# katie-jones/compressor-mpc

Measured on AMD Instinct MI355X. Metric: QP solves/sec (whole node), cooperative-parallel MPC, horizon p=50, higher is better.
Workload: dtype f64

## Files before the change

### compressor-mpc_amd/csrc/build_pair_kernel.h

```cpp
#pragma once
#include <hip/hip_runtime.h>
#include <stdint.h>

#include <algorithm>

#include "dispatch.h"
#include "rows_blocks.inc"

#ifndef CMPC_PAIR_ZDEPTH
#define CMPC_PAIR_ZDEPTH 1
#endif
static_assert(CMPC_PAIR_ZDEPTH == 1 || CMPC_PAIR_ZDEPTH == 2, "CMPC_PAIR_ZDEPTH");

__device__ __forceinline__ void pair_wait_dma() {
  asm volatile("" ::: "memory");
  __builtin_amdgcn_s_waitcnt(0x0F70);
  asm volatile("" ::: "memory");
}

template <int NS, int NY, int NUT, int NU, int M, int ND>
__global__ __launch_bounds__(64 * CMPC_BUILD_WAVES) __attribute__((amdgpu_waves_per_eu(2, 2)))
void cmpc_build_pair_kernel(BuildParams P) {
  extern __shared__ __attribute__((aligned(16))) double smem[];
  constexpr int WPG = CMPC_BUILD_WAVES;
  constexpr int NV = NU * M;
  constexpr int NC = M * NUT;
  constexpr int NG = NC + 2;
  constexpr int U = cmpc_rows_unroll(NY);
  constexpr int NCMP = CMPC_PAIR_CMP;
  static_assert(U == 5, "the unrolled block has 5 steps");
  static_assert(M == 2 && ND == 2 && NUT == 2 * NU, "two sub-controllers, two delayed inputs");
  static_assert(NG <= 16 && NS + NUT <= 16 && NS + NY + ND <= 16, "lane budget");
  const int lane = threadIdx.x & 63;
  const int wave = __builtin_amdgcn_readfirstlane(threadIdx.x >> 6);
  const int R = lane >> 4, j = lane & 15;
  const int pp = P.p, nobs = P.nobs, rl = P.rec_len, ndist = P.ndist;
  const int LQ = P.rows.LQ, WL = P.pair.WL, yls = P.rows.yls;
  const int nscn = P.nqp >> 1;
  const int ngroups = (nscn + 3) / 4;
  const int nwaves = gridDim.x * WPG;

  double* zeros = smem;
  double* ylT = smem + P.rows.yl_off;
  double* lw_all = smem + P.rows.lw_off;
  double* uw_all = smem + P.rows.uw_off;
  double* wreg = smem + P.rows.lds_block + wave * P.pair.per_wave;
  double* lines = wreg;
  double* chs = wreg + P.rows.ch_off;
  double* z1s = wreg + P.pair.z1_off;
  double* wtab = wreg + P.pair.w_off;

  const int nthr = 64 * WPG;
  for (int e = threadIdx.x; e < 2 * NY * yls; e += nthr) {
    const int ss = e / (NY * yls), rem = e - ss * NY * yls;
    const int o = rem / yls, r = rem - o * yls;
    ylT[e] = (r < pp) ? -P.cfg[(size_t)ss * P.co.len + P.co.yhat + r * NY + o] : 0.0;
  }
  for (int e = threadIdx.x; e < 2 * NY * NY; e += nthr)
    lw_all[e] = P.cfg[(size_t)(e / (NY * NY)) * P.co.len + P.co.lwt + e % (NY * NY)];
  for (int e = threadIdx.x; e < 2 * NU * NU; e += nthr)
    uw_all[e] = P.cfg[(size_t)(e / (NU * NU)) * P.co.len + P.co.uwt + e % (NU * NU)];
  if (threadIdx.x < 16) zeros[threadIdx.x] = 0.0;
  for (int e = lane; e < P.pair.per_wave; e += 64) wreg[e] = 0.0;
  if (blockIdx.x == 0 && threadIdx.x == 0) *P.pair_cnt_next = 0u;
  __syncthreads();

  const bool st = j < NS;
  const bool mk = j >= NS && j < NS + NUT;
  const int cm = mk ? j - NS : 0;
  const bool ol = j >= NS && j < NS + NY;
  const int oo = ol ? j - NS : 0;
  const bool cl = j >= 16 - ND;
  const int kc = cl ? j - (16 - ND) : 0;
  const bool gl = j < NG;
  const bool zl0 = j == NC, zl1 = j == NC + 1, zlane = zl0 || zl1;
  const int gk = (gl && !zlane) ? j / NUT : 0;
  const int gc = (gl && !zlane) ? j - gk * NUT : 0;
  const double smask = (gl && !zlane && gk == M - 1) ? 1.0 : 0.0;
  int dg = 0, dm = 0, log_ = 0, lom = 0, dinp[ND], dlen[ND], boff[ND];
#pragma unroll
  for (int c = 0; c < NUT; ++c) {
    if (c == gc) { dg = P.delay[c]; log_ = P.rows.lo[c]; }
    if (c == cm) { dm = P.delay[c]; lom = P.rows.lo[c]; }
  }
#pragma unroll
  for (int k = 0; k < ND; ++k) {
    dinp[k] = P.dinput[k];
    dlen[k] = P.dlen[k];
    boff[k] = P.boff[k];
  }
  int ysw = -1;
#pragma unroll
  for (int k = 0; k < ND; ++k)
    if (cl && k == kc && dlen[k] < pp) ysw = dlen[k];
  const int nseg = P.rows.nseg;
  constexpr int NSEG = 2 * ND;
  int segb[NSEG];
#pragma unroll
  for (int i = 0; i < NSEG; ++i) segb[i] = P.rows.seg[i];
  double* const qlines = lines + R * LQ;
  const bool rdel = gl && !zlane && dg > 0;
  const int rsw = (rdel && dg < pp) ? dg : -1;
  double* const zrow = qlines + P.rows.zr_off;
  double* const r_start = !gl ? zrow
                          : zl0 ? qlines + P.rows.z_off
                          : zl1 ? z1s + R * U * NY
                          : (dg == 0) ? qlines + log_ + (1 - gk) * NY
                                      : zrow;
  double* const r_line = qlines + log_ + (M - 1 - gk) * NY;
  const bool wdel = mk && dm > 0;
  double* const dump = qlines + P.rows.dump_off;
  double* const w_start = !mk ? dump
                          : (dm == 0) ? qlines + lom + NY
                          : (pp - dm > 0) ? qlines + lom + (M - 1) * NY
                                          : dump;
  const int winc0 = (wdel && pp - dm > 0) ? NY : 0;
  const int wsw = (wdel && pp - dm > 0) ? pp - dm : -1;
  const bool tl = mk && dm == 0;
  double* const tq = qlines + lom;
  double* const zq0 = ol ? qlines + P.rows.z_off + oo : dump;
  double* const zq1 = ol ? z1s + R * U * NY + oo : dump;

  const int t0 = P.pair.tail0, wch = rl >> 1, tch = (rl - t0) >> 1, sps = 2 * rl - t0;
  const int hd = P.off_x;
  int pli[NCMP];
#pragma unroll
  for (int i = 0; i < NCMP; ++i) {
    const int idx = 64 * i + lane;
    pli[i] = idx;
    if (idx >= P.off_B && idx < P.off_C) {
      const int t = idx - P.off_B, l = t / NUT, c = t - l * NUT;
      pli[i] = P.off_B + l * NUT + (c + NU) % NUT;
    }
  }

  const int share = (ngroups + nwaves - 1) / nwaves;
  const int g_first = blockIdx.x * WPG + wave;
  int done_groups = 0;
  uint32_t shared_scn = 0;
  __builtin_amdgcn_s_setprio(3);
  for (int g = g_first; g < ngroups; g += nwaves) {
    {
      const int level = 3 - (4 * done_groups) / share;
      if (level <= 0) __builtin_amdgcn_s_setprio(0);
      else if (level == 1) __builtin_amdgcn_s_setprio(1);
      else if (level == 2) __builtin_amdgcn_s_setprio(2);
      ++done_groups;
    }
    const int scn = 4 * g + R;
    const bool qv = scn < nscn;
    const int scc = qv ? scn : nscn - 1;
    const int nsc = min(4, nscn - 4 * g);
    const double* gbase = P.lin + (size_t)8 * g * rl;
    auto stage = [&](int h) {
#pragma unroll
      for (int sc = 0; sc < 4; ++sc) {
        if (sc >= nsc) break;
        const double* rec = gbase + (2 * sc + h) * rl + 2 * lane;
        const double* tal = gbase + (2 * sc + 1 - h) * rl + t0 + 2 * lane;
        double* dst = wreg + sc * sps;
        auto* gp = (__attribute__((address_space(1))) void*)rec;
        auto* lp = (__attribute__((address_space(3))) void*)dst;
        if (wch >= 64) __builtin_amdgcn_global_load_lds(gp, lp, 16, 0, 0);
        else if (lane < wch) __builtin_amdgcn_global_load_lds(gp, lp, 16, 0, 0);
        if (wch >= 128) __builtin_amdgcn_global_load_lds(gp, lp, 16, 1024, 0);
        else if (lane < wch - 64) __builtin_amdgcn_global_load_lds(gp, lp, 16, 1024, 0);
        if (wch >= 192) __builtin_amdgcn_global_load_lds(gp, lp, 16, 2048, 0);
        else if (lane < wch - 128) __builtin_amdgcn_global_load_lds(gp, lp, 16, 2048, 0);
        if (lane < tch)
          __builtin_amdgcn_global_load_lds((__attribute__((address_space(1))) void*)tal,
                                           (__attribute__((address_space(3))) void*)(dst + rl), 16, 0, 0);
      }
    };
    const double* lwt = lw_all;

    asm volatile("s_waitcnt lgkmcnt(0)" ::: "memory");
    stage(0);
    uint64_t hv[4][NCMP];
#pragma unroll
    for (int sc = 0; sc < 4; ++sc) {
      const int scl = min(sc, nsc - 1);
#pragma unroll
      for (int i = 0; i < NCMP; ++i)
        hv[sc][i] = reinterpret_cast<const uint64_t*>(gbase + (2 * scl + 1) * rl + 64 * i)[(uint32_t)lane];
    }
    double uo[2][ND], dyr[2][NY];
#pragma unroll
    for (int s = 0; s < 2; ++s) {
#pragma unroll
      for (int k = 0; k < ND; ++k) uo[s][k] = P.u_old[(size_t)(2 * scc + s) * NUT + dinp[k]];
#pragma unroll
      for (int o2 = 0; o2 < NY; ++o2) dyr[s][o2] = 0.0;
    }
    if (P.dy_ref) {
      uint32_t qo = (uint32_t)(2 * scc) * NY;
      asm volatile("" : "+v"(qo));
#pragma unroll
      for (int s = 0; s < 2; ++s)
#pragma unroll
        for (int o2 = 0; o2 < NY; ++o2) dyr[s][o2] = P.dy_ref[qo + s * NY + o2];
    }
    pair_wait_dma();
    uint64_t diff = 0ull;
#pragma unroll
    for (int sc = 0; sc < 4; ++sc) {
      const uint64_t* s0 = reinterpret_cast<const uint64_t*>(wreg + min(sc, nsc - 1) * sps);
#pragma unroll
      for (int i = 0; i < NCMP; ++i) {
        const uint64_t x = hv[sc][i] ^ s0[pli[i]];
        diff |= (64 * i + lane < hd) ? x : 0ull;
      }
    }
    const bool mism = __ballot(diff != 0ull) != 0ull;
    if (!mism) shared_scn += (uint32_t)nsc;

    for (int h = 0;; ++h) {
      int jg = j, Rg = R;
      asm volatile("" : "+v"(jg), "+v"(Rg));
      double* chq = chs + Rg * NY * 16;
      const double* srec = wreg + Rg * sps;
      const int rot = h * NU;
      const double *xa[2], *yv[2];
#pragma unroll
      for (int s = 0; s < 2; ++s) {
        const double* tb = (s == h) ? srec : srec + rl - t0;
        xa[s] = tb + P.off_x;
        yv[s] = tb + P.off_y;
      }
#pragma unroll
      for (int s = 0; s < 2; ++s)
#pragma unroll
        for (int k = 0; k < ND; ++k) {
          double* wk = wtab + ((Rg * 2 + s) * ND + k) * WL;
#pragma unroll
          for (int i = 0; i < 4; ++i) {
            const int t = jg + 16 * i;
            if (t < WL)
              wk[t] = (t < dlen[k]) ? ((t == 0) ? xa[s][ndist + k] : xa[s][boff[k] + t - 1]) - uo[s][k] : 0.0;
          }
        }
      double cs[NY];
#pragma unroll
      for (int o2 = 0; o2 < NY; ++o2) cs[o2] = (j < nobs) ? srec[P.off_C + o2 * nobs + jg] : 0.0;
      constexpr int KX = 16 - NS;
      double kx[2][KX], ky[2][NY];
#pragma unroll
      for (int s = 0; s < 2; ++s) {
#pragma unroll
        for (int d = 0; d < KX; ++d) kx[s][d] = (d < ndist) ? xa[s][d] : 0.0;
#pragma unroll
        for (int o2 = 0; o2 < NY; ++o2) ky[s][o2] = yv[s][o2];
#pragma unroll
        for (int o2 = 0; o2 < NY; ++o2) ky[s][o2] = ky[s][o2] - dyr[s][o2];
      }
      double mP[NS];
      if (st) {
        const double* src = srec + P.off_A + jg;
#pragma unroll
        for (int l = 0; l < NS; ++l) mP[l] = src[l * NS];
      } else if (mk) {
        const double* src = srec + P.off_B + (cm + rot) % NUT;
#pragma unroll
        for (int l = 0; l < NS; ++l) mP[l] = src[l * NUT];
      } else {
#pragma unroll
        for (int l = 0; l < NS; ++l) mP[l] = 0.0;
      }
      double mS[NS + ND], fj = 0.0;
      if (st) {
        const double* arow = srec + P.off_A + jg * NS;
        const double* brow = srec + P.off_B + jg * NUT;
#pragma unroll
        for (int l = 0; l < NS; ++l) mS[l] = arow[l];
#pragma unroll
        for (int k = 0; k < ND; ++k) mS[NS + k] = brow[(dinp[k] + rot) % NUT];
        fj = srec[P.off_f + jg];
      } else {
#pragma unroll
        for (int l = 0; l < NS + ND; ++l) mS[l] = 0.0;
      }
      __builtin_amdgcn_sched_barrier(0);

      double pP[NY];
#pragma unroll
      for (int o = 0; o < NY; ++o) {
        double t = 0.0;
#pragma unroll
        for (int o2 = 0; o2 < NY; ++o2)
          if (o2 >= o) t = __builtin_fma(lwt[o * NY + o2], cs[o2], t);
        if (j < nobs) chq[o * 16 + jg] = t;
        pP[o] = st ? t : 0.0;
      }
      double base0 = 0.0, base1 = 0.0, pS0 = 0.0, pS1 = 0.0, yh0 = 0.0, yh1 = 0.0;
      const double *yp0 = zeros, *yp1 = zeros;
      int yinc = 0;
      if (st) {
        base0 = base1 = fj;
        pS0 = pS1 = fj;
#pragma unroll
        for (int k = 0; k < ND; ++k) {
          pS0 = __builtin_fma(mS[NS + k], wtab[((Rg * 2 + 0) * ND + k) * WL], pS0);
          pS1 = __builtin_fma(mS[NS + ND - 1 - k], wtab[((Rg * 2 + 1) * ND + k) * WL], pS1);
        }
      } else if (ol) {
#pragma unroll
        for (int l = 0; l < NS; ++l) mS[l] = chq[oo * 16 + l];
        double t[2] = {0.0, 0.0};
#pragma unroll
        for (int s = 0; s < 2; ++s) {
#pragma unroll
          for (int d = 0; d < KX; ++d)
            if (d < ndist) t[s] = __builtin_fma(chq[oo * 16 + NS + d], kx[s][d], t[s]);
#pragma unroll
          for (int o2 = 0; o2 < NY; ++o2)
            if (o2 >= oo) t[s] = __builtin_fma(lwt[oo * NY + o2], ky[s][o2], t[s]);
        }
        base0 = t[0];
        base1 = t[1];
        const double* yl = ylT + oo * yls;
        yh0 = yl[0];
        yh1 = yl[NY * yls];
        yp0 = yl + 1;
        yp1 = yl + NY * yls + 1;
        yinc = 1;
      } else if (cl) {
        const double* wk0 = wtab + ((Rg * 2 + 0) * ND + kc) * WL;
        const double* wk1 = wtab + ((Rg * 2 + 1) * ND + (ND - 1 - kc)) * WL;
        pS0 = wk0[1];
        yh0 = wk0[2];
        yp0 = wk0 + 3;
        pS1 = wk1[1];
        yh1 = wk1[2];
        yp1 = wk1 + 3;
        yinc = 1;
      }
#pragma unroll
      for (int c = 0; c < NUT; ++c)
        if (P.delay[c] > 0 && j < (M - 1) * NY) qlines[P.rows.lo[c] + j] = 0.0;
      for (int e = j; e < U * NY; e += 16) qlines[P.rows.zr_off + e] = 0.0;
      if (tl) {
#pragma unroll
        for (int o = 0; o < NY; ++o) tq[o] = 0.0;
      }
      double cv[NY], rd[NY], acc[NC];
#pragma unroll
      for (int o = 0; o < NY; ++o) cv[o] = rd[o] = 0.0;
#pragma unroll
      for (int a = 0; a < NC; ++a) acc[a] = 0.0;
      double* wq = w_start;
      double* rq = r_start;
      int winc = winc0, rinc = 0;

#define CMPC_PAIR_STEP(u)                                                                  \
  {                                                                                        \
    double aS0 = aN0, aS1 = aN1;                                                           \
    yh0 = yp0[u];                                                                          \
    yh1 = yp1[u];                                                                          \
    double aP[NY];                                                                         \
    _Pragma("unroll") for (int o = 0; o < NY; ++o) aP[o] = z1[o];                          \
    rows_pair_head<NS, NY, ND, NUT, M>(pP, pS0, pS1, mP, mS, aP, aS0, aS1, cv, acc);       \
    __builtin_amdgcn_sched_barrier(0);                                                     \
    _Pragma("unroll") for (int o = 0; o < NY; ++o) cv[o] = __builtin_fma(smask, cv[o], rd[o]); \
    __builtin_amdgcn_sched_barrier(0);                                                     \
    rows_pair_part0<NS, NY, ND, NUT, M>(pP, pS0, pS1, mP, mS, aP, aS0, aS1, cv, acc);      \
    rows_pair_part1<NS, NY, ND, NUT, M>(pP, pS0, pS1, mP, mS, aP, aS0, aS1, cv, acc);      \
    __builtin_amdgcn_sched_barrier(0);                                                     \
    _Pragma("unroll") for (int o = 0; o < NY; ++o) pP[o] = aP[o];                          \
    pS0 = aS0;                                                                             \
    pS1 = aS1;                                                                             \
    if constexpr (CMPC_PAIR_ZDEPTH == 2) {                                                 \
      _Pragma("unroll") for (int o = 0; o < NY; ++o) z1[o] = z2[o];                        \
      _Pragma("unroll") for (int o = 0; o < NY; ++o) z2[o] = zeros[o];                     \
    } else {                                                                               \
      _Pragma("unroll") for (int o = 0; o < NY; ++o) z1[o] = zeros[o];                     \
    }                                                                                      \
    _Pragma("unroll") for (int o = 0; o < NY; ++o) wq[(u) * NY + o] = aP[o];               \
    zq0[(u) * NY] = aS0;                                                                   \
    zq1[(u) * NY] = aS1;                                                                   \
    _Pragma("unroll") for (int o = 0; o < NY; ++o) rd[o] = rq[(u) * NY + o];               \
    aN0 = base0 + yh0;                                                                     \
    aN1 = base1 + yh1;                                                                     \
    __builtin_amdgcn_sched_barrier(0);                                                     \
  }
#define CMPC_PAIR_TAIL()                                        \
  if (tl) {                                                     \
    _Pragma("unroll") for (int o = 0; o < NY; ++o) tq[o] = pP[o]; \
  }

      int r = 0;
      double aN0 = base0 + yh0, aN1 = base1 + yh1;
      double z1[NY], z2[NY];
#pragma unroll
      for (int o = 0; o < NY; ++o) z1[o] = z2[o] = zeros[o];
      for (int sg = 0; sg <= nseg; ++sg) {
        int r_end = pp;
#pragma unroll
        for (int i = 0; i < NSEG; ++i)
          if (i == sg && sg < nseg) r_end = segb[i];
        for (; r + U <= r_end; r += U) {
          CMPC_PAIR_STEP(0)
          CMPC_PAIR_STEP(1)
          CMPC_PAIR_STEP(2)
          CMPC_PAIR_STEP(3)
          CMPC_PAIR_STEP(4)
          CMPC_PAIR_TAIL()
          wq += U * winc;
          rq += U * rinc;
          yp0 += U * yinc;
          yp1 += U * yinc;
        }
        while (r + 2 <= r_end) {
          CMPC_PAIR_STEP(0)
          CMPC_PAIR_STEP(1)
          CMPC_PAIR_TAIL()
          wq += 2 * winc;
          rq += 2 * rinc;
          yp0 += 2 * yinc;
          yp1 += 2 * yinc;
          r += 2;
        }
        for (; r < r_end; ++r) {
          CMPC_PAIR_STEP(0)
          CMPC_PAIR_TAIL()
          wq += winc;
          rq += rinc;
          yp0 += yinc;
          yp1 += yinc;
        }
        if (r == rsw) { rq = r_line; rinc = NY; }
        if (r == wsw) { wq = dump; winc = 0; }
        if (r == ysw) { yp0 = yp1 = zeros; yinc = 0; }
      }
#undef CMPC_PAIR_STEP
#undef CMPC_PAIR_TAIL
#pragma unroll
      for (int o = 0; o < NY; ++o) cv[o] = __builtin_fma(smask, cv[o], rd[o]);
      rows_pair_gacc<NY, NUT, M>(cv, acc);

      if (qv && gl) {
        constexpr int nuo = NUT - NU, nVo = M * nuo;
        const int k2 = j / NUT, c2 = j - k2 * NUT;
#pragma unroll
        for (int s = 0; s < 2; ++s) {
          if (mism && s != h) continue;
          double* out = P.qp + (size_t)(2 * scn + s) * P.qp_len;
          const double* uwt = uw_all + s * NU * NU;
          double own[NV];
#pragma unroll
          for (int a = 0; a < NV; ++a) own[a] = acc[(a / NU) * NUT + (a % NU + s * NU) % NUT];
          if (zlane) {
            if (j == NC + s) {
#pragma unroll
              for (int a = 0; a < NV; ++a) out[NV * NV + a] = own[a];
            }
          } else {
            const int cs_ = (c2 + NUT - s * NU) % NUT;
            if (cs_ < NU) {
#pragma unroll
              for (int a = 0; a < NV; ++a) {
                const double rw = (a / NU == k2) ? uwt[(a % NU) * NU + cs_] : 0.0;
                out[a * NV + k2 * NU + cs_] = own[a] + rw;
              }
            } else {
#pragma unroll
              for (int a = 0; a < NV; ++a) out[NV * NV + NV + a * nVo + k2 * nuo + (cs_ - NU)] = own[a];
            }
          }
        }
      }
      __builtin_amdgcn_wave_barrier();
      if (!mism || h == 1) break;
      asm volatile("s_waitcnt lgkmcnt(0)" ::: "memory");
      stage(1);
      pair_wait_dma();
    }
  }
  if (lane == 0 && shared_scn) atomicAdd(P.pair_cnt, shared_scn);
}

template <int NS, int NY, int NU, int M>
static int pair_launch(const BuildParams& P, hipStream_t s) {
  auto kern = cmpc_build_pair_kernel<NS, NY, CMPC_DIMS_NUT, NU, M, CMPC_DIMS_ND>;
  constexpr int WPG = CMPC_BUILD_WAVES;
  const size_t lds = sizeof(double) * ((size_t)P.rows.lds_block + (size_t)P.pair.per_wave * WPG);
  if (lds > 64 * 1024) cmpc_allow_lds(reinterpret_cast<const void*>(kern), lds);
  const int per_cu = 2;
  const int nscn = P.nqp / 2;
  const int need = std::max(1, ((nscn + 3) / 4 + WPG - 1) / WPG);
  const int grid = std::max(1, std::min(need, P.cus * per_cu));
  cmpc_launch(kern, dim3(grid), dim3(64 * WPG), lds, s, P);
  return 0;
}
```

Before: 4.642 billion.

## Branch-free pair setup with hoisted loads and high priority during setup

Rewrites the per-half setup of the pair build kernel so it has no branches. Loads are issued with pointer selects, redirecting to a zero buffer or dump slot instead of using conditional paths, and all operand loads are hoisted ahead of a scheduling barrier so their latency overlaps. By default the wave now holds top priority through setup and only drops to its fair-share priority when the main row loop starts. The change also adds opt-in timing instrumentation and a next-group prefetch touch, both disabled by default. Risks are extra register pressure from hoisting and extra dummy stores.

Measured after the change: 4.792 billion (median of 6 runs). 3.2% higher.

```diff
diff --git a/compressor-mpc_amd/csrc/build_pair_kernel.h b/compressor-mpc_amd/csrc/build_pair_kernel.h
--- a/compressor-mpc_amd/csrc/build_pair_kernel.h
+++ b/compressor-mpc_amd/csrc/build_pair_kernel.h
@@ -11,6 +11,28 @@
 #define CMPC_PAIR_ZDEPTH 1
 #endif
 static_assert(CMPC_PAIR_ZDEPTH == 1 || CMPC_PAIR_ZDEPTH == 2, "CMPC_PAIR_ZDEPTH");
+
+#ifndef CMPC_PAIR_TIMING
+#define CMPC_PAIR_TIMING 0
+#endif
+#ifndef CMPC_PAIR_SETUP_PRIO
+#define CMPC_PAIR_SETUP_PRIO 1
+#endif
+#ifndef CMPC_PAIR_TOUCH
+#define CMPC_PAIR_TOUCH 0
+#endif
+#if CMPC_PAIR_TIMING
+#define CMPC_PT(i)                                         \
+  {                                                        \
+    __builtin_amdgcn_sched_barrier(0);                     \
+    const uint64_t now_ = __builtin_amdgcn_s_memtime();    \
+    tsum[i] += now_ - tlast;                               \
+    tlast = now_;                                          \
+    __builtin_amdgcn_sched_barrier(0);                     \
+  }
+#else
+#define CMPC_PT(i)
+#endif
 
 __device__ __forceinline__ void pair_wait_dma() {
   asm volatile("" ::: "memory");
@@ -138,36 +160,45 @@
   const int g_first = blockIdx.x * WPG + wave;
   int done_groups = 0;
   uint32_t shared_scn = 0;
+#if CMPC_PAIR_TIMING
+  uint64_t tsum[7] = {0, 0, 0, 0, 0, 0, 0}, tlast = __builtin_amdgcn_s_memtime();
+  const uint64_t t0c = tlast, t0r = __builtin_amdgcn_s_memrealtime();
+  int ngrp = 0;
+#endif
   __builtin_amdgcn_s_setprio(3);
+  float touch[3] = {0.f, 0.f, 0.f};
   for (int g = g_first; g < ngroups; g += nwaves) {
-    {
-      const int level = 3 - (4 * done_groups) / share;
+    CMPC_PT(6)
+    const int level = 3 - (4 * done_groups) / share;
+    ++done_groups;
+    auto fair_prio = [&]() {
       if (level <= 0) __builtin_amdgcn_s_setprio(0);
       else if (level == 1) __builtin_amdgcn_s_setprio(1);
       else if (level == 2) __builtin_amdgcn_s_setprio(2);
-      ++done_groups;
-    }
+    };
+    if (CMPC_PAIR_SETUP_PRIO) __builtin_amdgcn_s_setprio(3);
+    else fair_prio();
     const int scn = 4 * g + R;
     const bool qv = scn < nscn;
     const int scc = qv ? scn : nscn - 1;
     const int nsc = min(4, nscn - 4 * g);
     const double* gbase = P.lin + (size_t)8 * g * rl;
-    auto stage = [&](int h) {
+    auto stage = [&](int h, int ln) {
 #pragma unroll
       for (int sc = 0; sc < 4; ++sc) {
         if (sc >= nsc) break;
-        const double* rec = gbase + (2 * sc + h) * rl + 2 * lane;
-        const double* tal = gbase + (2 * sc + 1 - h) * rl + t0 + 2 * lane;
+        const double* rec = gbase + (2 * sc + h) * rl + 2 * ln;
+        const double* tal = gbase + (2 * sc + 1 - h) * rl + t0 + 2 * ln;
         double* dst = wreg + sc * sps;
         auto* gp = (__attribute__((address_space(1))) void*)rec;
         auto* lp = (__attribute__((address_space(3))) void*)dst;
         if (wch >= 64) __builtin_amdgcn_global_load_lds(gp, lp, 16, 0, 0);
-        else if (lane < wch) __builtin_amdgcn_global_load_lds(gp, lp, 16, 0, 0);
+        else if (ln < wch) __builtin_amdgcn_global_load_lds(gp, lp, 16, 0, 0);
         if (wch >= 128) __builtin_amdgcn_global_load_lds(gp, lp, 16, 1024, 0);
-        else if (lane < wch - 64) __builtin_amdgcn_global_load_lds(gp, lp, 16, 1024, 0);
+        else if (ln < wch - 64) __builtin_amdgcn_global_load_lds(gp, lp, 16, 1024, 0);
         if (wch >= 192) __builtin_amdgcn_global_load_lds(gp, lp, 16, 2048, 0);
-        else if (lane < wch - 128) __builtin_amdgcn_global_load_lds(gp, lp, 16, 2048, 0);
-        if (lane < tch)
+        else if (ln < wch - 128) __builtin_amdgcn_global_load_lds(gp, lp, 16, 2048, 0);
+        if (ln < tch)
           __builtin_amdgcn_global_load_lds((__attribute__((address_space(1))) void*)tal,
                                            (__attribute__((address_space(3))) void*)(dst + rl), 16, 0, 0);
       }
@@ -175,7 +206,7 @@
     const double* lwt = lw_all;
 
     asm volatile("s_waitcnt lgkmcnt(0)" ::: "memory");
-    stage(0);
+    stage(0, lane);
     uint64_t hv[4][NCMP];
 #pragma unroll
     for (int sc = 0; sc < 4; ++sc) {
@@ -200,7 +231,10 @@
 #pragma unroll
         for (int o2 = 0; o2 < NY; ++o2) dyr[s][o2] = P.dy_ref[qo + s * NY + o2];
     }
+    CMPC_PT(0)
     pair_wait_dma();
+    CMPC_PT(1)
+    if (CMPC_PAIR_TOUCH) asm volatile("" ::"v"(touch[0]), "v"(touch[1]), "v"(touch[2]));
     uint64_t diff = 0ull;
 #pragma unroll
     for (int sc = 0; sc < 4; ++sc) {
@@ -213,6 +247,7 @@
     }
     const bool mism = __ballot(diff != 0ull) != 0ull;
     if (!mism) shared_scn += (uint32_t)nsc;
+    CMPC_PT(2)
 
     for (int h = 0;; ++h) {
       int jg = j, Rg = R;
@@ -227,6 +262,67 @@
         xa[s] = tb + P.off_x;
         yv[s] = tb + P.off_y;
       }
+      static_assert(U * NY <= 16, "one zero-restore store per lane");
+      static_assert((NUT & (NUT - 1)) == 0, "column rotation by a mask");
+      const int oog = ol ? jg - NS : 0, kcg = cl ? jg - (16 - ND) : 0, cmg = mk ? jg - NS : 0;
+      double wv[2][ND][4];
+      bool wlive[ND][4];
+#pragma unroll
+      for (int k = 0; k < ND; ++k)
+#pragma unroll
+        for (int i = 0; i < 4; ++i) {
+          const int t = jg + 16 * i;
+          wlive[k][i] = t < WL && t < dlen[k];
+          const int src = (wlive[k][i] && t > 0) ? boff[k] + t - 1 : ndist + k;
+#pragma unroll
+          for (int s = 0; s < 2; ++s) wv[s][k][i] = xa[s][src];
+        }
+      const bool jo = j < nobs;
+      double cs[NY];
+      {
+        const double* src = jo ? srec + P.off_C + jg : zeros;
+        const int str = jo ? nobs : 0;
+#pragma unroll
+        for (int o2 = 0; o2 < NY; ++o2) cs[o2] = src[o2 * str];
+      }
+      constexpr int KX = 16 - NS;
+      double kx[2][KX], ky[2][NY];
+#pragma unroll
+      for (int s = 0; s < 2; ++s) {
+#pragma unroll
+        for (int d = 0; d < KX; ++d) kx[s][d] = xa[s][(d < ndist) ? d : 0];
+#pragma unroll
+        for (int o2 = 0; o2 < NY; ++o2) ky[s][o2] = yv[s][o2];
+      }
+      double mP[NS];
+      {
+        const double* src = st ? srec + P.off_A + jg : mk ? srec + P.off_B + ((cmg + rot) & (NUT - 1)) : zeros;
+        const int str = st ? NS : mk ? NUT : 0;
+#pragma unroll
+        for (int l = 0; l < NS; ++l) mP[l] = src[l * str];
+      }
+      double ma[NS], mb[ND], fj;
+      {
+        const double* arow = st ? srec + P.off_A + jg * NS : zeros;
+        const double* brow = st ? srec + P.off_B + jg * NUT : zeros;
+        const double* frow = st ? srec + P.off_f + jg : zeros;
+#pragma unroll
+        for (int l = 0; l < NS; ++l) ma[l] = arow[l];
+#pragma unroll
+        for (int k = 0; k < ND; ++k) mb[k] = brow[(dinp[k] + rot) % NUT];
+        fj = *frow;
+      }
+      double lu[NY][NY];
+#pragma unroll
+      for (int o = 0; o < NY; ++o)
+#pragma unroll
+        for (int o2 = o; o2 < NY; ++o2) lu[o][o2] = lwt[o * NY + o2];
+      __builtin_amdgcn_sched_barrier(0);
+#pragma unroll
+      for (int s = 0; s < 2; ++s)
+#pragma unroll
+        for (int o2 = 0; o2 < NY; ++o2) ky[s][o2] = ky[s][o2] - dyr[s][o2];
+
 #pragma unroll
       for (int s = 0; s < 2; ++s)
 #pragma unroll
@@ -235,113 +331,81 @@
 #pragma unroll
           for (int i = 0; i < 4; ++i) {
             const int t = jg + 16 * i;
-            if (t < WL)
-              wk[t] = (t < dlen[k]) ? ((t == 0) ? xa[s][ndist + k] : xa[s][boff[k] + t - 1]) - uo[s][k] : 0.0;
+            double* dst = wlive[k][i] ? wk + t : dump;
+            *dst = wv[s][k][i] - uo[s][k];
           }
         }
-      double cs[NY];
-#pragma unroll
-      for (int o2 = 0; o2 < NY; ++o2) cs[o2] = (j < nobs) ? srec[P.off_C + o2 * nobs + jg] : 0.0;
-      constexpr int KX = 16 - NS;
-      double kx[2][KX], ky[2][NY];
-#pragma unroll
-      for (int s = 0; s < 2; ++s) {
-#pragma unroll
-        for (int d = 0; d < KX; ++d) kx[s][d] = (d < ndist) ? xa[s][d] : 0.0;
-#pragma unroll
-        for (int o2 = 0; o2 < NY; ++o2) ky[s][o2] = yv[s][o2];
-#pragma unroll
-        for (int o2 = 0; o2 < NY; ++o2) ky[s][o2] = ky[s][o2] - dyr[s][o2];
-      }
-      double mP[NS];
-      if (st) {
-        const double* src = srec + P.off_A + jg;
-#pragma unroll
-        for (int l = 0; l < NS; ++l) mP[l] = src[l * NS];
-      } else if (mk) {
-        const double* src = srec + P.off_B + (cm + rot) % NUT;
-#pragma unroll
-        for (int l = 0; l < NS; ++l) mP[l] = src[l * NUT];
-      } else {
-#pragma unroll
-        for (int l = 0; l < NS; ++l) mP[l] = 0.0;
-      }
-      double mS[NS + ND], fj = 0.0;
-      if (st) {
-        const double* arow = srec + P.off_A + jg * NS;
-        const double* brow = srec + P.off_B + jg * NUT;
-#pragma unroll
-        for (int l = 0; l < NS; ++l) mS[l] = arow[l];
-#pragma unroll
-        for (int k = 0; k < ND; ++k) mS[NS + k] = brow[(dinp[k] + rot) % NUT];
-        fj = srec[P.off_f + jg];
-      } else {
-#pragma unroll
-        for (int l = 0; l < NS + ND; ++l) mS[l] = 0.0;
-      }
-      __builtin_amdgcn_sched_barrier(0);
-
+      CMPC_PT(3)
       double pP[NY];
 #pragma unroll
       for (int o = 0; o < NY; ++o) {
         double t = 0.0;
 #pragma unroll
         for (int o2 = 0; o2 < NY; ++o2)
-          if (o2 >= o) t = __builtin_fma(lwt[o * NY + o2], cs[o2], t);
-        if (j < nobs) chq[o * 16 + jg] = t;
+          if (o2 >= o) t = __builtin_fma(lu[o][o2], cs[o2], t);
+        chq[o * 16 + jg] = t;
         pP[o] = st ? t : 0.0;
       }
-      double base0 = 0.0, base1 = 0.0, pS0 = 0.0, pS1 = 0.0, yh0 = 0.0, yh1 = 0.0;
-      const double *yp0 = zeros, *yp1 = zeros;
-      int yinc = 0;
-      if (st) {
-        base0 = base1 = fj;
-        pS0 = pS1 = fj;
-#pragma unroll
-        for (int k = 0; k < ND; ++k) {
-          pS0 = __builtin_fma(mS[NS + k], wtab[((Rg * 2 + 0) * ND + k) * WL], pS0);
-          pS1 = __builtin_fma(mS[NS + ND - 1 - k], wtab[((Rg * 2 + 1) * ND + k) * WL], pS1);
-        }
-      } else if (ol) {
-#pragma unroll
-        for (int l = 0; l < NS; ++l) mS[l] = chq[oo * 16 + l];
-        double t[2] = {0.0, 0.0};
-#pragma unroll
-        for (int s = 0; s < 2; ++s) {
-#pragma unroll
-          for (int d = 0; d < KX; ++d)
-            if (d < ndist) t[s] = __builtin_fma(chq[oo * 16 + NS + d], kx[s][d], t[s]);
-#pragma unroll
-          for (int o2 = 0; o2 < NY; ++o2)
-            if (o2 >= oo) t[s] = __builtin_fma(lwt[oo * NY + o2], ky[s][o2], t[s]);
-        }
-        base0 = t[0];
-        base1 = t[1];
-        const double* yl = ylT + oo * yls;
-        yh0 = yl[0];
-        yh1 = yl[NY * yls];
-        yp0 = yl + 1;
-        yp1 = yl + NY * yls + 1;
-        yinc = 1;
-      } else if (cl) {
-        const double* wk0 = wtab + ((Rg * 2 + 0) * ND + kc) * WL;
-        const double* wk1 = wtab + ((Rg * 2 + 1) * ND + (ND - 1 - kc)) * WL;
-        pS0 = wk0[1];
-        yh0 = wk0[2];
-        yp0 = wk0 + 3;
-        pS1 = wk1[1];
-        yh1 = wk1[2];
-        yp1 = wk1 + 3;
-        yinc = 1;
-      }
-#pragma unroll
-      for (int c = 0; c < NUT; ++c)
-        if (P.delay[c] > 0 && j < (M - 1) * NY) qlines[P.rows.lo[c] + j] = 0.0;
-      for (int e = j; e < U * NY; e += 16) qlines[P.rows.zr_off + e] = 0.0;
-      if (tl) {
-#pragma unroll
-        for (int o = 0; o < NY; ++o) tq[o] = 0.0;
-      }
+
+      const double* yl = ylT + oog * yls;
+      const double* wk0 = cl ? wtab + ((Rg * 2 + 0) * ND + kcg) * WL : zeros;
+      const double* wk1 = cl ? wtab + ((Rg * 2 + 1) * ND + (ND - 1 - kcg)) * WL : zeros;
+      double ch[16], lw[NY], w0[2][ND];
+#pragma unroll
+      for (int l = 0; l < 16; ++l) ch[l] = chq[oog * 16 + l];
+#pragma unroll
+      for (int o2 = 0; o2 < NY; ++o2) lw[o2] = lwt[oog * NY + o2];
+#pragma unroll
+      for (int s = 0; s < 2; ++s)
+#pragma unroll
+        for (int k = 0; k < ND; ++k) w0[s][k] = wtab[((Rg * 2 + s) * ND + k) * WL];
+      const double yl0 = yl[0], yl1 = yl[NY * yls];
+      const double c01 = wk0[1], c02 = wk0[2], c11 = wk1[1], c12 = wk1[2];
+      double z1[NY], z2[NY];
+#pragma unroll
+      for (int o = 0; o < NY; ++o) z1[o] = z2[o] = zeros[o];
+#pragma unroll
+      for (int c = 0; c < NUT; ++c) {
+        double* dst = (P.delay[c] > 0 && jg < (M - 1) * NY) ? qlines + P.rows.lo[c] + jg : dump;
+        *dst = 0.0;
+      }
+      qlines[P.rows.zr_off + min(jg, U * NY - 1)] = 0.0;
+#pragma unroll
+      for (int o = 0; o < NY; ++o) {
+        double* dst = tl ? tq + o : dump;
+        *dst = 0.0;
+      }
+      double x0 = fj, x1 = fj;
+#pragma unroll
+      for (int k = 0; k < ND; ++k) {
+        x0 = __builtin_fma(mb[k], w0[0][k], x0);
+        x1 = __builtin_fma(mb[ND - 1 - k], w0[1][k], x1);
+      }
+      double kap[2] = {0.0, 0.0};
+#pragma unroll
+      for (int s = 0; s < 2; ++s) {
+#pragma unroll
+        for (int d = 0; d < KX; ++d) {
+          const double tn = __builtin_fma(ch[NS + d], kx[s][d], kap[s]);
+          kap[s] = (d < ndist) ? tn : kap[s];
+        }
+#pragma unroll
+        for (int o2 = 0; o2 < NY; ++o2) {
+          const double tn = __builtin_fma(lw[o2], ky[s][o2], kap[s]);
+          kap[s] = (o2 >= oog) ? tn : kap[s];
+        }
+      }
+      double mS[NS + ND];
+#pragma unroll
+      for (int l = 0; l < NS; ++l) mS[l] = ol ? ch[l] : ma[l];
+#pragma unroll
+      for (int k = 0; k < ND; ++k) mS[NS + k] = mb[k];
+      const double base0 = ol ? kap[0] : fj, base1 = ol ? kap[1] : fj;
+      double pS0 = st ? x0 : c01, pS1 = st ? x1 : c11;
+      double yh0 = ol ? yl0 : c02, yh1 = ol ? yl1 : c12;
+      const double* yp0 = ol ? yl + 1 : wk0 + 3;
+      const double* yp1 = ol ? yl + NY * yls + 1 : wk1 + 3;
+      int yinc = (ol || cl) ? 1 : 0;
       double cv[NY], rd[NY], acc[NC];
 #pragma unroll
       for (int o = 0; o < NY; ++o) cv[o] = rd[o] = 0.0;
@@ -389,10 +453,17 @@
 
       int r = 0;
       double aN0 = base0 + yh0, aN1 = base1 + yh1;
-      double z1[NY], z2[NY];
-#pragma unroll
-      for (int o = 0; o < NY; ++o) z1[o] = z2[o] = zeros[o];
+      CMPC_PT(4)
+      if (CMPC_PAIR_SETUP_PRIO) fair_prio();
       for (int sg = 0; sg <= nseg; ++sg) {
+        if (CMPC_PAIR_TOUCH && sg == nseg) {
+          const int gn = (g + nwaves < ngroups) ? g + nwaves : g;
+          const char* nb = reinterpret_cast<const char*>(P.lin + (size_t)8 * gn * rl);
+          const int nbytes = 2 * min(4, nscn - 4 * gn) * rl * (int)sizeof(double);
+#pragma unroll
+          for (int i = 0; i < 3; ++i)
+            touch[i] = *reinterpret_cast<const float*>(nb + min((lane + 64 * i) * 128, nbytes - 4));
+        }
         int r_end = pp;
 #pragma unroll
         for (int i = 0; i < NSEG; ++i)
@@ -436,20 +507,26 @@
 #pragma unroll
       for (int o = 0; o < NY; ++o) cv[o] = __builtin_fma(smask, cv[o], rd[o]);
       rows_pair_gacc<NY, NUT, M>(cv, acc);
-
-      if (qv && gl) {
+#if CMPC_PAIR_TIMING
+#pragma unroll
+      for (int a = 0; a < NC; ++a) asm volatile("" ::"v"(acc[a]));
+#endif
+      CMPC_PT(5)
+
+      if (qv && gl && !CMPC_PAIR_TIMING) {
         constexpr int nuo = NUT - NU, nVo = M * nuo;
-        const int k2 = j / NUT, c2 = j - k2 * NUT;
+        const int k2 = jg / NUT, c2 = jg - k2 * NUT;
+        const int scg = 4 * g + Rg;
 #pragma unroll
         for (int s = 0; s < 2; ++s) {
           if (mism && s != h) continue;
-          double* out = P.qp + (size_t)(2 * scn + s) * P.qp_len;
+          double* out = P.qp + (size_t)(2 * scg + s) * P.qp_len;
           const double* uwt = uw_all + s * NU * NU;
           double own[NV];
 #pragma unroll
           for (int a = 0; a < NV; ++a) own[a] = acc[(a / NU) * NUT + (a % NU + s * NU) % NUT];
           if (zlane) {
-            if (j == NC + s) {
+            if (jg == NC + s) {
 #pragma unroll
               for (int a = 0; a < NV; ++a) out[NV * NV + a] = own[a];
             }
@@ -469,13 +546,35 @@
         }
       }
       __builtin_amdgcn_wave_barrier();
+      CMPC_PT(6)
       if (!mism || h == 1) break;
       asm volatile("s_waitcnt lgkmcnt(0)" ::: "memory");
-      stage(1);
+      int l1 = lane;
+      asm volatile("" : "+v"(l1));
+      stage(1, l1);
       pair_wait_dma();
+      CMPC_PT(1)
     }
+#if CMPC_PAIR_TIMING
+    ++ngrp;
+#endif
   }
   if (lane == 0 && shared_scn) atomicAdd(P.pair_cnt, shared_scn);
+#if CMPC_PAIR_TIMING
+  const size_t wid = (size_t)blockIdx.x * WPG + wave;
+  if (lane == 0 && (wid + 1) * 16 <= (size_t)P.nqp * P.qp_len) {
+    const uint64_t t1c = __builtin_amdgcn_s_memtime(), t1r = __builtin_amdgcn_s_memrealtime();
+    double* dbg = P.qp + wid * 16;
+    for (int i = 0; i < 7; ++i) dbg[i] = (double)tsum[i];
+    dbg[7] = 1.0;
+    dbg[8] = (double)(t1c - t0c);
+    dbg[9] = (double)(t1r - t0r);
+    dbg[10] = (double)t0r;
+    dbg[11] = (double)t1r;
+    dbg[12] = (double)ngrp;
+    dbg[13] = (double)wid;
+  }
+#endif
 }
 
 template <int NS, int NY, int NU, int M>
```
